# XiaoJiang-Phy/TensorCrossInterpolation.jl

Hardware: AMD Instinct MI355X
Metric: rrLU GFLOP/s at (m,n,r)=(8192,8192,256) (higher is better)
Workload: dtype f64

## Files before the change

include/tci_hip.h:

```cpp
#ifndef TCI_HIP_H
#define TCI_HIP_H

#include <stdint.h>

#ifdef __cplusplus
extern "C" {
#endif

#define TCI_OK 0
#define TCI_ERR_ARG 1
#define TCI_ERR_NAN 2
#define TCI_ERR_NONSQ 3
#define TCI_ERR_DEVICE 4
#define TCI_ERR_NOMEM 5
#define TCI_ERR_HOST 6

#define TCI_F_SUM 0
#define TCI_F_LORENTZ 1
#define TCI_F_TABLE 2
#define TCI_F_GAUSS 3
#define TCI_F_GAUSSMIX 4
#define TCI_F_QOSC 5
#define TCI_F_QEXP 6
#define TCI_F_TT 7
// ... 10 lines not shown
typedef int (*tci_exchange_fn)(void* user, int op, const void* d_send, void* d_recv, int64_t count);

int tci_ctx_create(int device, tci_ctx** out);
int tci_ctx_destroy(tci_ctx* ctx);
const char* tci_last_error(const tci_ctx* ctx);
void* tci_ctx_stream(tci_ctx* ctx);
int tci_ctx_synchronize(tci_ctx* ctx);
int tci_last_kernel_stats(tci_ctx* ctx, int family, double* total_ms, int64_t* launches);
int tci_last_kernel_units(tci_ctx* ctx, int family, double* total_ms, int64_t* launches, int64_t* units);
int tci_set_timing(tci_ctx* ctx, int enabled);
int tci_set_rrlu_flush(tci_ctx* ctx, int nb);
int tci_set_rrlu_epochs(tci_ctx* ctx, int epochs);
int tci_rrlu_epochs_for(tci_ctx* ctx, int64_t m, int64_t n);
int tci_set_rrlu_small(tci_ctx* ctx, int enabled);
int tci_set_rrlu_mid(tci_ctx* ctx, int enabled);
int tci_set_rrlu_persist(tci_ctx* ctx, int enabled);
int tci_rrlu_persist_faulted(tci_ctx* ctx);
int tci_set_shard_exchange(tci_ctx* ctx, int mode);
int tci_last_shard_exchange(tci_ctx* ctx);
int tci_set_rrlu_shadow(tci_ctx* ctx, int enabled);
int tci_rrlu_shadow_bytes(void);
int tci_set_c128_shadow(tci_ctx* ctx, int enabled);

int tci_set_dense_mfma(tci_ctx* ctx, int mask);

int tci_func_create(tci_ctx* ctx, int kind, const double* params, int64_t nparams,
                    const int32_t* localdims, int32_t L, tci_func** out);
int tci_func_destroy(tci_func* f);

typedef int (*tci_host_fn)(void* user, const int32_t* I, int64_t m, int32_t nl, const int32_t* J,
// ... 181 lines not shown
```

tensorcrossinterpolation.jl_amd/csrc/tci_abi.cpp:

```cpp
#include <hip/hip_runtime.h>
#include <stdint.h>
#include <stdlib.h>
#include <string.h>

#include <algorithm>
#include <cstddef>
#include <cmath>
#include <string>
#include <thread>
#include <vector>

#include <rccl/rccl.h>

#include "../../include/tci_hip.h"
#include "tci_internal.h"

using tci::Cand;
using tci::FuncDev;
using tci::RrluState;

struct tci_ctx {
    int device = 0;
    hipStream_t stream = nullptr;
    std::string err;
// ... 10 lines not shown
    double* xbuf = nullptr;
    size_t capX = 0;
    double* ybuf = nullptr;
    size_t capY = 0;
    int flush_every = 10;
    int epochs = 0;
    int serpentine = 1;
    int shadow = 1;
    int pass_gridx = 1;
    int pass_griddiv = 1;
    float* sbuf = nullptr;
    size_t capS = 0;
    int small_path = 1;
    int mid_path = 1;
    int mid_faulted = 0;
    int persist = 0;
    int persist_faulted = 0;
    int persist_kinds = 3;
    int persist_maxpass = 1 << 30;
    unsigned* esync = nullptr;
    size_t capEsync = 0;
    int dense = tci::kDenseAll;
    int c128_nb = -1;
    int c128_sh = 1;
    int ncu = 0;
    double* colbuf = nullptr;
    size_t capColbuf = 0;
    unsigned* bar = nullptr;
    int* fault = nullptr;
    int* flag = nullptr;
// ... 516 lines not shown
    g.lds = 0;
    if (shadow) {
        g.lds = round_up(m, 16);
        if ((st = ensure(c, &c->sbuf, &c->capS, (size_t)(g.lds * n)))) return st;
        g.S = c->sbuf;
        if ((st = zero_shadow_pad(c, g.lds, m, n))) return st;
    }
    const int grid = tci::argmax_grid(mi, ni, -1, g.cb,
                                      std::min(std::max(std::max(c->ncu, 1) * c->pass_gridx / c->pass_griddiv, 8), kMaxGrid));
    const int epochs = (shadow && tci::shadow_two_level() && nb >= 2 && nb <= 15 &&
                        tci::refresh_fits(g.lds, n))
                           ? std::max(1, std::min(rrlu_epochs(c, m, n), tci::kMaxPendR / nb)) : 1;
    const int nbx = nb * epochs;
    g.nbs = nb;
    g.pe = g.ps = 0;
    g.Asrc = dsrc;
    g.ldsrc = ldsrc;
    tci::launch_pass(c->stream, 0, false, shadow, g, grid);
    g.Asrc = nullptr;
    struct Sched {
        int PE, PS;
        bool last, flush, refresh;
    };
    auto sched = [&](int64_t kk, int64_t te, int64_t ts) {
        Sched s;
        s.PE = (int)(kk - te) + 1;
        s.PS = (int)(kk - ts) + 1;
        s.last = kk + 1 >= mr;
        s.flush = s.PE >= nbx && !s.last;
        s.refresh = !s.flush && epochs > 1 && s.PS >= nb && !s.last;
        return s;
    };
// ... 4 lines not shown
    int64_t nlaunch = 0;
    if (persist) {
        const size_t slots = (size_t)mr / 2 + 2;
        if ((st = ensure(c, &c->esync, &c->capEsync, slots * tci::kEpochSlot))) return st;
        HIPCHK(c, hipMemsetAsync(c->esync, 0, slots * tci::kEpochSlot * sizeof(unsigned), c->stream));
    }
    int64_t k = 0, chunk = 2, te = 0, ts = 0;
    StopPoll poll(c, c->st);
    for (;;) {
        while (k < mr) {
            const int64_t kend = std::min<int64_t>(k + chunk, mr);
            int64_t kk = k;
            while (kk < kend) {
                const Sched s = sched(kk, te, ts);
                const bool ro = !s.flush && !s.refresh && !s.last;
                if (persist && ro && kk >= 1 && s.PS <= tci::kEpochMaxP && (c->persist_kinds & (s.PE > s.PS ? 2 : 1))) {
                    int np = 1;
                    for (; np < c->persist_maxpass; ++np) {
                        const Sched t = sched(kk + np, te, ts);
                        if (t.flush || t.refresh || t.last || t.PS > tci::kEpochMaxP) break;
                    }
                    if (np >= 2) {
                        g.k = (int)kk;
                        g.pe = s.PE;
                        g.ps = s.PS;
                        g.selk = (int)(kk + 1);
                        const bool sampled = nlaunch % 3 == 0;
                        ev_begin(c, s.PE > s.PS ? tci_ctx::kFamEpoch + 1 : tci_ctx::kFamEpoch, sampled, -1, np);
                        tci::launch_pass_epoch(c->stream, g, grid, np, c->serpentine,
                                               c->esync + (size_t)nlaunch * tci::kEpochSlot, ptimeout);
// ... 33 lines not shown
        persist = false;
        k = c->hst->np - 1;
        te = ts = 0;
        for (int64_t q = 0; q < k; ++q) {
            const Sched s = sched(q, te, ts);
            if (s.flush) te = ts = q + 1;
            if (s.refresh) ts = q + 1;
        }
        HIPCHK(c, hipMemsetAsync(&c->st->done, 0, sizeof(int32_t), c->stream));
        chunk = 2;
        poll = StopPoll(c, c->st);
    }
    int64_t np = c->hst->np;
    double err = c->hst->error;
    if (np >= std::min(m, n)) err = 0.0;
    *np_out = np;
    *err_out = err;
    return TCI_OK;
}

int extract_LU(tci_ctx* c, int64_t m, int64_t n, int64_t np, int leftorth, bool wantL, bool wantU) {
    if (np <= 0) return TCI_OK;
    int st;
    if (wantL && (st = ensure(c, &c->dL, &c->capL, (size_t)(m * np)))) return st;
    if (wantU && (st = ensure(c, &c->dU, &c->capU, (size_t)(np * n)))) return st;
    HIPCHK(c, hipMemsetAsync(c->flag, 0, sizeof(int), c->stream));
    tci::launch_extract(c->stream, c->Lp, m, c->Up, c->ldUp, c->pivv, c->rowperm, c->colperm, (int)m,
                        (int)n, (int)np, leftorth, wantL ? c->dL : nullptr, m, wantU ? c->dU : nullptr,
                        np, c->flag);
    HIPCHK(c, hipMemcpyAsync(c->hflag, c->flag, sizeof(int), hipMemcpyDeviceToHost, c->stream));
// ... 322 lines not shown
    if (hipGetDeviceCount(&ndev) != hipSuccess || ndev <= 0) return TCI_ERR_DEVICE;
    if (device < 0 || device >= ndev) return TCI_ERR_ARG;
    tci_ctx* c = new tci_ctx();
    c->device = device;
    if (const char* e = getenv("TCI_RRLU_NB")) c->flush_every = std::max(1, std::min(atoi(e), tci::kMaxPend));
    if (const char* e = getenv("TCI_RRLU_SERP")) c->serpentine = atoi(e) != 0;
    if (const char* e = getenv("TCI_RRLU_EPOCHS")) c->epochs = std::max(0, std::min(atoi(e), tci::kMaxPendR));
    if (const char* e = getenv("TCI_RRLU_SHADOW")) c->shadow = atoi(e) != 0;
    if (const char* e = getenv("TCI_PASS_GRIDX")) c->pass_gridx = std::max(1, std::min(atoi(e), 8));
    if (const char* e = getenv("TCI_PASS_GRIDDIV")) c->pass_griddiv = std::max(1, std::min(atoi(e), 16));
    if (const char* e = getenv("TCI_RRLU_SMALL")) c->small_path = atoi(e) != 0;
    if (const char* e = getenv("TCI_SWEEP_SMALL")) c->small_sweep = atoi(e) != 0;
    if (const char* e = getenv("TCI_SW_LUWAVE")) c->sw_lu_wave = atoi(e) != 0;
    if (const char* e = getenv("TCI_SW_LAZYU")) c->sw_lazy_union = atoi(e) != 0;
    if (const char* e = getenv("TCI_RRLU_MID")) c->mid_path = atoi(e) != 0;
    if (const char* e = getenv("TCI_RRLU_PERSIST")) c->persist = tci::kEpochGrid && atoi(e) != 0;
    if (const char* e = getenv("TCI_SHARD_EXCHANGE")) c->sh_exchange = std::max(0, std::min(atoi(e), 2));
    if (const char* e = getenv("TCI_EPOCH_KINDS")) c->persist_kinds = atoi(e);
    if (const char* e = getenv("TCI_EPOCH_MAXPASS")) c->persist_maxpass = std::max(1, atoi(e));
    if (const char* e = getenv("TCI_C128_NB")) c->c128_nb = std::max(0, std::min(atoi(e), tci::kMaxPend - 1));
    if (const char* e = getenv("TCI_C128_SH")) c->c128_sh = atoi(e) != 0;
    if (const char* e = getenv("TCI_DENSE_MFMA")) c->dense = std::max(0, std::min(atoi(e), (int)tci::kDenseAll));
    {
        hipDeviceProp_t prop;
        if (hipGetDeviceProperties(&prop, device) == hipSuccess) c->ncu = prop.multiProcessorCount;
    }
    if (hipSetDevice(device) != hipSuccess ||
        hipStreamCreateWithFlags(&c->stream, hipStreamNonBlocking) != hipSuccess) {
        delete c;
        return TCI_ERR_DEVICE;
// ... 100 lines not shown

int tci_set_c128_shadow(tci_ctx* c, int enabled) {
    c->c128_sh = enabled != 0;
    return TCI_OK;
}

int tci_set_dense_mfma(tci_ctx* c, int mask) {
    if (!c || mask < 0 || mask > tci::kDenseAll) return TCI_ERR_ARG;
    c->dense = mask;
    return TCI_OK;
}

int tci_set_rrlu_mid(tci_ctx* c, int enabled) {
    c->mid_path = enabled != 0;
    c->mid_faulted = 0;
    return TCI_OK;
}

int tci_set_rrlu_persist(tci_ctx* c, int enabled) {
    if (!c) return TCI_ERR_ARG;
    if (enabled < 0 || enabled > 2) return set_err(c, TCI_ERR_ARG, "persist must be 0, 1 or 2 (test mode)");
    if (enabled && !tci::kEpochGrid)
        return set_err(c, TCI_ERR_ARG, "the persistent epoch grid is not built (default; -DTCI_EPOCH_GRID=1)");
    c->persist = enabled;
    c->persist_faulted = 0;
    return TCI_OK;
}

int tci_rrlu_persist_faulted(tci_ctx* c) { return c ? c->persist_faulted : -1; }

// ... 1796 lines not shown
```

tensorcrossinterpolation.jl_amd/csrc/tci_rrlu.hip:

```cpp
#include <hip/hip_runtime.h>
#include <math.h>
#include <stdint.h>

#include <type_traits>

#include "tci_internal.h"
#include "tci_smalllu.h"

#ifndef TCI_PASS2_U
#define TCI_PASS2_U 4
#endif
#ifndef TCI_SH_HALF
#define TCI_SH_HALF 1
#endif
#ifndef TCI_PASS_SH_U
#define TCI_PASS_SH_U 2
#endif
#ifndef TCI_SH_MFMA
#define TCI_SH_MFMA TCI_SH_HALF
#endif
#ifndef TCI_SH_NT
#define TCI_SH_NT 0
#endif
#ifndef TCI_SH_TIGHT
// ... 506 lines not shown
template <bool COH, typename T>
__device__ __forceinline__ T ldc(const T* p) {
    if constexpr (COH)
        return __hip_atomic_load((gptr<T>)(p), __ATOMIC_RELAXED, __HIP_MEMORY_SCOPE_AGENT);
    else
        return *p;
}
template <bool COH, typename T>
__device__ __forceinline__ void stc(T* p, T v) {
    if constexpr (COH)
        __hip_atomic_store((gptr<T>)(p), v, __ATOMIC_RELAXED, __HIP_MEMORY_SCOPE_AGENT);
    else
        *p = v;
}

template <int P, bool FLUSH, bool SH, bool COH = false>
__device__ __forceinline__ bool pass2_body(const PassK& g, const SelArgs& sel,
                                           P2Lds<(P > 0 ? P : 1)>& L, CandR& best,
                                           unsigned long long (&pt)[8]) {
    RrluState* st = sel.st;
    const int32_t* rowpos = sel.rowpos;
    const int32_t* colpos = sel.colpos;
    double* __restrict__ A = g.A;
    const int64_t lda = g.lda;
    const int m = g.m, n = g.n, k = g.k, cb = g.cb, rev = g.rev, leftorth = g.leftorth;
    double* __restrict__ X = g.X;
    double* __restrict__ Y = g.Y;
    const int64_t ldx = g.ldx, ldy = g.ldy;
    constexpr int U = TCI_PASS2_U;
    static_assert(U <= 8 && 8 % U == 0, "U must divide every column-tile width");
    constexpr int PP = P > 0 ? P : 1;
// ... 1 lines not shown
    int* cpos_s = L.cpos;
    int* cnt = L.cnt;
    const int lane = threadIdx.x & 63, wave = threadIdx.x >> 6;
    const int slice = wave % kP2Slices, rep = wave / kP2Slices;
    const int tiles_r = (m + kRowsPerTile - 1) / kRowsPerTile;
    const int tiles_c = (n + cb - 1) / cb;
    const int nq = gridDim.x / tiles_r;
    const int wid = xcd_spread(blockIdx.x, gridDim.x);
    const int tr = wid % tiles_r;
    const int q = rev ? nq - 1 - wid / tiles_r : wid / tiles_r;
    const int ntc = q < tiles_c ? (tiles_c - 1 - q) / nq + 1 : 0;
    const int G = kP2StageCols / cb;
    const int r0 = tr * kRowsPerTile + slice * 128 + 2 * lane;
    const bool rowok = r0 < m, pair = r0 + 1 < m;
    double* const base = A + (rowok ? r0 : 0);
    const bool cpy = P == 0 && g.Asrc != nullptr;
    const double* const sbase = cpy ? g.Asrc + (rowok ? r0 : 0) : base;
    const int64_t slda = cpy ? g.ldsrc : lda;
    auto chunk_col = [&](int g0, int h) -> int {
        const int it = g0 + (h * U) / cb;
        return (q + (rev ? ntc - 1 - it : it) * nq) * cb + (h * U) % cb;
    };
    auto load_chunk = [&](int g0, int h, double2 (&v)[U]) {
        const int j = chunk_col(g0, h);
#pragma unroll
        for (int u = 0; u < U; ++u) {
            const double2* pa = reinterpret_cast<const double2*>(sbase + (int64_t)min(j + u, n - 1) * slda);
            if constexpr (FLUSH && TCI_FLUSH_NTL) {
                typedef double dv2 __attribute__((ext_vector_type(2)));
                const dv2 w = __builtin_nontemporal_load(reinterpret_cast<const dv2*>(pa));
                v[u] = double2{w.x, w.y};
// ... 27 lines not shown
    if (rep < nch0) load_chunk(0, rep, va);
    if (rep + kP2Reps < nch0) load_chunk(0, rep + kP2Reps, vb);
    if (st->done) return false;
    int a = 0, b = 0;
    double piv = 1.0;
    if (P > 0) {
        a = (int)st->p;
        b = (int)st->q;
        piv = st->pval;
    }
    const bool in0 = rp0 > k, in1 = rp1 > k;
    const bool active = in0 || in1;
    [[maybe_unused]] const double shs =
        (SH && kShHalf && P > 0) ? sh_scale(sh_bound(sel.pivvals, FLUSH ? k + 1 : 0)) : 1.0;
    if constexpr (P > 0) {
        const double2 cb2 = *reinterpret_cast<const double2*>(A + (rowok ? r0 : 0) + (int64_t)b * lda);
        double xk0 = cb2.x, xk1 = cb2.y;
#pragma unroll
        for (int s = 0; s < P - 1; ++s) {
            const double yv = Y[(int64_t)s * ldy + b];
            xk0 = __dsub_rn(xk0, __dmul_rn(x0[s], yv));
            xk1 = __dsub_rn(xk1, __dmul_rn(x1[s], yv));
        }
        if (leftorth) {
            xk0 = xk0 / piv;
            xk1 = xk1 / piv;
        }
        x0[P - 1] = xk0;
        x1[P - 1] = xk1;
        if (q == 0 && rep == 0) {
            double* xs = X + (int64_t)(P - 1) * ldx;
            if (in0) {
                stc<COH>(xs + r0, xk0);
                g.Lp[r0 + (int64_t)k * g.ldl] = xk0;
            }
            if (in1) {
                stc<COH>(xs + r0 + 1, xk1);
                g.Lp[r0 + 1 + (int64_t)k * g.ldl] = xk1;
            }
        }
    }
    PPROF(1);
    const bool wact = (SH && kShHalf && P > 0) || __any(active);
    for (int g0 = 0; g0 < ntc; g0 += G) {
        const int gn = min(G, ntc - g0);
        const int nch = gn * cb / U;
        if (g0 > 0) {
            jst = stage_col(g0);
            cpst = (jst >= 0 && jst < n) ? colpos[jst] : -1;
            if (wact) {
                if (rep < nch) load_chunk(g0, rep, va);
                if (rep + kP2Reps < nch) load_chunk(g0, rep + kP2Reps, vb);
            }
            __syncthreads();
        }
        if (jst >= 0) {
            const int lc = threadIdx.x;
            cpos_s[lc] = cpst;
            if (P > 0 && cpst > k) {
                double yk = A[a + (int64_t)jst * lda];
#pragma unroll
                for (int s = 0; s < P - 1; ++s) {
                    const double ysv = Y[(int64_t)s * ldy + jst];
                    ys[lc * PP + s] = ysv;
                    yk = __dsub_rn(yk, __dmul_rn(X[(int64_t)s * ldx + a], ysv));
                }
                if (!leftorth) yk = yk / piv;
                ys[lc * PP + P - 1] = yk;
                if (tr == 0) {
                    stc<COH>(Y + (int64_t)(P - 1) * ldy + jst, yk);
                    g.Up[k + (int64_t)jst * g.ldu] = yk;
                }
            }
        }
        if (threadIdx.x < kP2Slices) cnt[threadIdx.x] = 2 * kP2Reps;
        __syncthreads();
        if (g0 == 0) PPROF(2);
        if (!wact) continue;
        auto column = [&](double2 v, int lc, int j) {
            const int cp = cpos_s[lc];
            if (cp <= k) return;
            if (P == 0 && cpy && rowok) {
                double* pw = base + (int64_t)j * lda;
                if (pair)
                    *reinterpret_cast<double2*>(pw) = v;
                else
                    pw[0] = v.x;
            }
            if constexpr (SH && kShHalf && !FLUSH && P > 0) {
                if (rowok && kShU8) {
                    uint8_t* ps = reinterpret_cast<uint8_t*>(g.S) + r0 + (int64_t)j * g.lds;
                    const uint32_t c0 = sh_u8((float)(v.x * shs));
                    if (pair)
                        *reinterpret_cast<uint16_t*>(ps) = (uint16_t)(c0 | sh_u8((float)(v.y * shs)) << 8);
                    else
                        ps[0] = (uint8_t)c0;
// ... 80 lines not shown
        };
        int h0 = rep, h1 = rep + kP2Reps;
        while (h0 < nch) {
            process(h0, va);
            h0 = grab();
            if (h0 < nch) load_chunk(g0, h0, va);
            if (h1 >= nch) break;
            process(h1, vb);
            h1 = grab();
            if (h1 < nch) load_chunk(g0, h1, vb);
        }
    }
    return true;
}

template <int P, bool FLUSH, bool SH>
__global__ __launch_bounds__(kP2Threads) void k_pass2(PassK g, SelArgs sel) {
    __shared__ P2Lds<(P > 0 ? P : 1)> L;
    [[maybe_unused]] unsigned long long pt[8] = {0, 0, 0, 0, 0, 0, 0, 0};
    PPROF(0);
    CandR best = cand_none();
    if (!pass2_body<P, FLUSH, SH>(g, sel, L, best, pt)) return;
    PPROF(3);
    pass_tail<kP2Threads>(best, sel, g.cand, pt, g.m, P, (int)FLUSH);
}

template <int P>
__device__ __forceinline__ bool pass_sh_body(const PassK& g, const SelArgs& sel, P2Lds<P>& L,
                                             CandR& best, float eps, double shs,
                                             unsigned long long (&pt)[8]) {
    RrluState* st = sel.st;
    const int32_t* colpos = sel.colpos;
    const int m = g.m, n = g.n, k = g.k, cb = g.cb, rev = g.rev;
    const int64_t lda = g.lda, ldx = g.ldx, ldy = g.ldy, lds = g.lds;
    constexpr int U = TCI_PASS_SH_U;
    const int lane = threadIdx.x & 63, wave = threadIdx.x >> 6;
    const int slice = wave % kShSlices, rep = wave / kShSlices;
// ... 978 lines not shown

constexpr int kXHalf = 256;
#ifndef TCI_XSTAGE
#define TCI_XSTAGE 128
#endif
#ifndef TCI_PX_EXP
#define TCI_PX_EXP 0
#endif
constexpr int kXStage = TCI_XSTAGE;
#ifndef TCI_PX_DRAIN
#define TCI_PX_DRAIN 1
#endif
#ifndef TCI_XU
#define TCI_XU 4
#endif
constexpr int kXU = TCI_XU;
static_assert(kXU == 4 || kXU == 8, "chunks of 4 or 8 columns (cb is a multiple of 8)");
constexpr int kXSlices = kXHalf / 128;
constexpr int kXReps = kP2Threads / 64 / kXSlices;
template <int NT>
struct PxGeom {
    static constexpr int Half = NT == 1024 ? 256 : 128;
    static constexpr int Tile = 2 * Half;
    static constexpr int Slices = Half / 128;
    static constexpr int Reps = NT / 64 / Slices;
};
template <int NT>
struct alignas(16) PxLdsT {
    alignas(16) double xs[kMaxPendR * PxGeom<NT>::Half];
    alignas(16) double ys[kMaxPendR * kXStage];
    double xa[kMaxPendR];
    double yb[kMaxPendR];
    int cpos[kXStage];
    int cnt[PxGeom<NT>::Slices];
};
using PxLds = PxLdsT<kP2Threads>;

template <int MODE, bool COH = false, int NT = kP2Threads>
__device__ __forceinline__ bool passx_body(const PassK& g, const SelArgs& sel, PxLdsT<NT>& L, CandR& best,
                                           unsigned long long (&pt)[8]) {
    constexpr int kXHalf = PxGeom<NT>::Half, kXSlices = PxGeom<NT>::Slices, kXReps = PxGeom<NT>::Reps;
    constexpr int kRowsPerTile = PxGeom<NT>::Tile, kP2Threads = NT;
    RrluState* st = sel.st;
    const int32_t* rowpos = sel.rowpos;
    const int32_t* colpos = sel.colpos;
    double* __restrict__ A = g.A;
    const int64_t lda = g.lda, ldx = g.ldx, ldy = g.ldy;
    const int m = g.m, n = g.n, k = g.k, cb = g.cb, rev = g.rev, leftorth = g.leftorth;
    const int P = g.pe;
    const int lane = threadIdx.x & 63, wave = __builtin_amdgcn_readfirstlane(threadIdx.x >> 6);
    const int slice = wave % kXSlices, rep = wave / kXSlices;
    const int tiles_r = (m + kRowsPerTile - 1) / kRowsPerTile;
    const int tiles_c = (n + cb - 1) / cb;
    const int nq = gridDim.x / tiles_r;
    const int wid = xcd_spread(blockIdx.x, gridDim.x);
    const int tr = wid % tiles_r;
    const int q = rev ? nq - 1 - wid / tiles_r : wid / tiles_r;
    const int ntc = q < tiles_c ? (tiles_c - 1 - q) / nq + 1 : 0;
    const int G = kXStage / cb;
    const int cbs = __builtin_ctz(cb);
    auto col_of = [&](int g0, int lc) -> int {
        const int it = g0 + (lc >> cbs);
// ... 20 lines not shown
                const int e = threadIdx.x + u * kP2Threads, s = e / kXHalf, rr = e - s * kXHalf;
                v[u] = g.X[(int64_t)s * ldx + min(hb + rr, m - 1)];
                if (!(s < P - 1 && hb + rr < m)) v[u] = 0.0;
            }
#pragma unroll
            for (int u = 0; u < kPer; ++u) {
                const int e = threadIdx.x + u * kP2Threads;
                if (e < (P - 1) * kXHalf) L.xs[e] = v[u];
            }
        }
        __syncthreads();
        if (threadIdx.x < kXHalf) {
            const int rr = threadIdx.x, r = hb + rr;
            double xk = 0.0;
            if (r < m) {
                xk = A[r + (int64_t)b * lda];
                for (int s = 0; s < P - 1; ++s) xk = __dsub_rn(xk, __dmul_rn(L.xs[s * kXHalf + rr], L.yb[s]));
                if (leftorth) xk = xk / piv;
                if (q == 0 && rowpos[r] > k) {
                    stc<COH>(g.X + (int64_t)(P - 1) * ldx + r, xk);
                    g.Lp[r + (int64_t)k * g.ldl] = xk;
                }
            }
            L.xs[(P - 1) * kXHalf + rr] = xk;
        }
        const int lr = slice * 128 + 2 * lane;
        const int r0 = hb + lr;
        const bool rowok = r0 < m, pair = r0 + 1 < m;
        const int rp0 = rowok ? rowpos[r0] : -1, rp1 = pair ? rowpos[r0 + 1] : -1;
        const bool in0 = rp0 > k, in1 = rp1 > k;
        const bool wact = MODE != 0 || __any(in0 || in1);
// ... 9 lines not shown
                double v[kPer];
#pragma unroll
                for (int u = 0; u < kPer; ++u) {
                    const int s = s0 + u * (kP2Threads / kXStage);
                    v[u] = g.Y[(int64_t)s * ldy + j];
                    if (!(s < P - 1 && lc < gcols)) v[u] = 0.0;
                }
#pragma unroll
                for (int u = 0; u < kPer; ++u) {
                    const int s = s0 + u * (kP2Threads / kXStage);
                    if (s < P - 1) L.ys[s * kXStage + lc] = v[u];
                }
            }
            const int lcs = threadIdx.x, js = lcs < gcols ? col_of(g0, lcs) : 0;
            const int cps = (lcs < gcols && js < n) ? colpos[js] : -1;
            const double ypr = (lcs < gcols && cps > k) ? A[a + (int64_t)js * lda] : 0.0;
            __syncthreads();
            if (lcs < gcols) {
                L.cpos[lcs] = cps;
                if (cps > k) {
                    double yk = ypr;
                    for (int s = 0; s < P - 1; ++s) yk = __dsub_rn(yk, __dmul_rn(L.xa[s], L.ys[s * kXStage + lcs]));
                    if (!leftorth) yk = yk / piv;
                    L.ys[(P - 1) * kXStage + lcs] = yk;
                    if (tr == 0 && half == 0) {
                        stc<COH>(g.Y + (int64_t)(P - 1) * ldy + js, yk);
                        g.Up[k + (int64_t)js * g.ldu] = yk;
                    }
                }
            }
            if (threadIdx.x < kXSlices) L.cnt[threadIdx.x] = 2 * kXReps;
            __syncthreads();
            if (g0 == 0 && half == 0) PPROF(2);
            if (!wact) continue;
            auto load_chunk = [&](int h, double2 (&v)[kXU]) {
                const int j0 = col_of(g0, h * kXU);
#pragma unroll
                for (int u = 0; u < kXU; ++u) {
                    const double* colp = A + (int64_t)min(j0 + u, n - 1) * lda;
                    const double2* pa = reinterpret_cast<const double2*>(colp + roff);
                    if constexpr (MODE == 1 && TCI_FLUSH_NTL) {
                        typedef double dv2 __attribute__((ext_vector_type(2)));
                        const dv2 w = __builtin_nontemporal_load(reinterpret_cast<const dv2*>(pa));
                        v[u] = double2{w.x, w.y};
                    } else {
                        v[u] = *pa;
                    }
                }
            };
            auto process = [&](int h, double2 (&v)[kXU]) {
                int cp[kXU];
                bool any = false;
#pragma unroll
                for (int u = 0; u < kXU; ++u) {
                    cp[u] = __builtin_amdgcn_readfirstlane(L.cpos[h * kXU + u]);
                    any |= cp[u] > k;
                }
                if (!any) return;
                const int j0 = col_of(g0, h * kXU);
#pragma unroll 2
                for (int s = 0; s < P; ++s) {
#if TCI_PX_EXP & 1
                    const dv2 x = dv2{1.0 + s, 0.5 * s};
#else
                    const dv2 x = *reinterpret_cast<const dv2*>(
                        __builtin_assume_aligned(&L.xs[s * kXHalf + lr], 16));
#endif
                    double y[kXU];
#pragma unroll
                    for (int u = 0; u < kXU; u += 2) {
#if TCI_PX_EXP & 2
// ... 5 lines not shown
                        y[u] = yy.x;
                        y[u + 1] = yy.y;
                    }
#pragma unroll
                    for (int u = 0; u < kXU; ++u) {
                        v[u].x = __dsub_rn(v[u].x, __dmul_rn(x.x, y[u]));
                        v[u].y = __dsub_rn(v[u].y, __dmul_rn(x.y, y[u]));
                    }
                }
                double mx0 = 0.0, mx1 = 0.0;
#pragma unroll
                for (int u = 0; u < kXU; ++u) {
                    if (cp[u] <= k) continue;
                    const int j = j0 + u;
                    if constexpr (MODE == 1) {
                        if (in0 || in1) {
                            double2* pa = reinterpret_cast<double2*>(A + (int64_t)j * lda + roff);
                            if (!in1) {
                                pa->x = v[u].x;
                            } else if (!in0) {
                                pa->y = v[u].y;
                            } else {
                                typedef double dv2 __attribute__((ext_vector_type(2)));
                                dv2 w = {v[u].x, v[u].y};
                                __builtin_nontemporal_store(w, reinterpret_cast<dv2*>(pa));
                            }
                        }
                    }
                    if constexpr (MODE != 0 && kShU8) {
                        if (rowok) {
                            uint8_t* ps = reinterpret_cast<uint8_t*>(g.S) + (int64_t)j * g.lds + roff;
                            const uint32_t c0 = in0 ? sh_u8((float)(v[u].x * shs)) : kShU8Zero;
                            if (pair)
                                *reinterpret_cast<uint16_t*>(ps) =
                                    (uint16_t)(c0 | (in1 ? sh_u8((float)(v[u].y * shs)) : kShU8Zero) << 8);
                            else
// ... 54 lines not shown
            while (h0 < nch) {
                process(h0, va);
                h0 = grab();
                if (h0 < nch) load_chunk(h0, va);
                if (h1 >= nch) break;
                process(h1, vb);
                h1 = grab();
                if (h1 < nch) load_chunk(h1, vb);
            }
#endif
        }
    }
    return true;
}

template <int MODE, int NT = kP2Threads>
__global__ __launch_bounds__(NT) __attribute__((amdgpu_waves_per_eu(4))) void k_pass_x(PassK g, SelArgs sel) {
    __shared__ PxLdsT<NT> L;
    [[maybe_unused]] unsigned long long pt[8] = {0, 0, 0, 0, 0, 0, 0, 0};
    PPROF(0);
    CandR best = cand_none();
    if (!passx_body<MODE, false, NT>(g, sel, L, best, pt)) return;
    PPROF(3);
    pass_tail<NT>(best, sel, g.cand, pt, g.m, g.pe, MODE);
}

template <int P, bool EXT, bool RF, bool RT = false>
__global__ __launch_bounds__(kP2Threads) void k_pass_mf(PassK g, SelArgs sel) {
    __shared__ union {
        P2Lds<P> x;
        P2MfLds<P, EXT> f;
        typename std::conditional<(EXT || RF), PxLds, char>::type px;
    } L;
    [[maybe_unused]] unsigned long long pt[8] = {0, 0, 0, 0, 0, 0, 0, 0};
    PPROF(0);
#if TCI_PASS_PROF
    if (threadIdx.x == 0) g_exam_lds = 0;
// ... 209 lines not shown
}

int shadow_elem_bytes() { return kShU8 ? 1 : kShHalf ? 2 : 4; }
bool shadow_two_level() { return kShHalf && TCI_SH_MFMA; }

int argmax_grid(int m, int n, int k, int cb, int max_grid) {
    (void)k;
    const long long tiles_r = m > 0 ? (m + kRowsPerTile - 1) / kRowsPerTile : 1;
    const long long tiles_c = n > 0 ? (n + cb - 1) / cb : 1;
    long long nq = max_grid / tiles_r;
    if (nq > tiles_c) nq = tiles_c;
    if (nq < 1) nq = 1;
    return (int)(tiles_r * nq);
}

template <int P>
static void launch_pass_p(hipStream_t s, bool flush, bool shadow, const PassArgs& g, int grid, int kind) {
    const SelArgs sel{g.rowpos, g.colpos, g.rowphys, g.colphys, g.pivvals, g.st,
                      g.ticket, g.reltol, g.abstol,  g.selk,    g.lout, g.pc_off};
    const PassK a{g.A,  g.lda, g.m,  g.n,   g.k,        g.X,    g.ldx, g.Y,   g.ldy,
                  g.Lp, g.ldl, g.Up, g.ldu, g.leftorth, g.cand, g.cb,  g.rev, g.S, g.lds,
                  g.pe, g.ps, g.nbs, g.Asrc, g.ldsrc};
    if (shadow && kShHalf) {
        if (P == 0)
            hipLaunchKernelGGL((k_pass2<0, false, false>), dim3(grid), dim3(kP2Threads), 0, s, a, sel);
        else if (flush)
            hipLaunchKernelGGL((k_pass2<P, true, true>), dim3(grid), dim3(kP2Threads), 0, s, a, sel);
        else if (P == 1 && g.k == 0)
            hipLaunchKernelGGL((k_pass2<1, false, true>), dim3(grid), dim3(kP2Threads), 0, s, a, sel);
        else if constexpr (P > 0) {
            const bool ext = g.pe > g.ps, rf = kind == 2;
            if constexpr (TCI_SH_MFMA && P <= kMfMaxP) {
                if (ext && rf)
                    hipLaunchKernelGGL((k_pass_mf<P, true, true>), dim3(grid), dim3(kP2Threads), 0, s, a, sel);
                else if (ext && TCI_PASS_ONEP)
                    hipLaunchKernelGGL((k_pass_mf<kEpochMaxP, true, false, true>), dim3(grid), dim3(kP2Threads), 0, s, a, sel);
                else if (ext)
                    hipLaunchKernelGGL((k_pass_mf<P, true, false>), dim3(grid), dim3(kP2Threads), 0, s, a, sel);
                else if (rf)
                    hipLaunchKernelGGL((k_pass_mf<P, false, true>), dim3(grid), dim3(kP2Threads), 0, s, a, sel);
                else
                    hipLaunchKernelGGL((k_pass_mf<P, false, false>), dim3(grid), dim3(kP2Threads), 0, s, a, sel);
            } else if constexpr (kShU8) {
// ... 4 lines not shown
        }
    } else if (shadow && !kShHalf) {
        if constexpr (!kShHalf) {
            if (flush || P == 0)
                hipLaunchKernelGGL((k_pass2<P, (P > 0), true>), dim3(grid), dim3(kP2Threads), 0, s, a, sel);
            else if constexpr (P > 0)
                hipLaunchKernelGGL((k_pass_sh<P>), dim3(grid), dim3(kP2Threads), 0, s, a, sel);
        }
    } else if (flush) {
        hipLaunchKernelGGL((k_pass2<P, true, false>), dim3(grid), dim3(kP2Threads), 0, s, a, sel);
    } else {
        hipLaunchKernelGGL((k_pass2<P, false, false>), dim3(grid), dim3(kP2Threads), 0, s, a, sel);
    }
}

#ifndef TCI_PASSX_MIN
#define TCI_PASSX_MIN 12
#endif

void launch_pass(hipStream_t s, int P, bool flush, bool shadow, const PassArgs& g, int grid, int kind) {
    if (kind < 0) kind = flush ? 1 : 0;
    PassArgs h = g;
    if (h.pe <= 0) h.pe = h.ps = P;
    if (kind == 1 && shadow && kShHalf && h.pe >= TCI_PASSX_MIN) {
        const SelArgs sel{h.rowpos, h.colpos, h.rowphys, h.colphys, h.pivvals, h.st,
                          h.ticket, h.reltol, h.abstol,  h.selk,    h.lout, h.pc_off};
        const PassK a{h.A,  h.lda, h.m,  h.n,   h.k,        h.X,    h.ldx, h.Y,   h.ldy,
                      h.Lp, h.ldl, h.Up, h.ldu, h.leftorth, h.cand, h.cb,  h.rev, h.S, h.lds,
                      h.pe, h.ps, h.nbs, h.Asrc, h.ldsrc};
        static const int px_nt = [] {
            const char* e = getenv("TCI_PASSX_NT");
            return e ? atoi(e) : 512;
        }();
        const int tiles_r = (h.m + kRowsPerTile - 1) / kRowsPerTile;
        const int nq = grid / tiles_r;
        const int tiles_r2 = (h.m + PxGeom<512>::Tile - 1) / PxGeom<512>::Tile;
        if (px_nt == 512 && (int64_t)tiles_r2 * nq <= kMaxPassGrid)
            hipLaunchKernelGGL((k_pass_x<1, 512>), dim3(tiles_r2 * nq), dim3(512), 0, s, a, sel);
        else
            hipLaunchKernelGGL((k_pass_x<1>), dim3(grid), dim3(kP2Threads), 0, s, a, sel);
        return;
    }
    const int PP = kind == 1 || !(shadow && kShHalf) ? h.pe : h.ps;
    switch (PP) {
#define TCI_PASS_CASE(p) \
    case p: launch_pass_p<p>(s, kind == 1, shadow, h, grid, kind); break;
        TCI_PASS_CASE(0) TCI_PASS_CASE(1) TCI_PASS_CASE(2) TCI_PASS_CASE(3) TCI_PASS_CASE(4)
        TCI_PASS_CASE(5) TCI_PASS_CASE(6) TCI_PASS_CASE(7) TCI_PASS_CASE(8) TCI_PASS_CASE(9)
        TCI_PASS_CASE(10) TCI_PASS_CASE(11) TCI_PASS_CASE(12) TCI_PASS_CASE(13) TCI_PASS_CASE(14)
        TCI_PASS_CASE(15) TCI_PASS_CASE(16)
#undef TCI_PASS_CASE
    default: break;
// ... 662 lines not shown
```

tensorcrossinterpolation.jl_amd/tci_amd/_lib.py:

```python
import atexit
import ctypes as C
import os
import threading
import weakref

import numpy as np

_HERE = os.path.dirname(os.path.abspath(__file__))
LIB_PATH = os.environ.get("TCI_HIP_LIB", os.path.join(os.path.dirname(_HERE), "lib", "libtci_hip.so"))

TCI_OK, TCI_ERR_ARG, TCI_ERR_NAN, TCI_ERR_NONSQ, TCI_ERR_DEVICE, TCI_ERR_NOMEM, TCI_ERR_HOST = range(7)

i64p = np.ctypeslib.ndpointer(dtype=np.int64, flags="C_CONTIGUOUS")
i32p = np.ctypeslib.ndpointer(dtype=np.int32, flags="C_CONTIGUOUS")
f64p = np.ctypeslib.ndpointer(dtype=np.float64, flags="C_CONTIGUOUS")
vp = C.c_void_p
dbl = C.c_double
i64 = C.c_int64
i32 = C.c_int32
pi64 = C.POINTER(C.c_int64)
pdbl = C.POINTER(C.c_double)


class TCIError(RuntimeError):
# ... 17 lines not shown
    "tci_last_error": ([vp], C.c_char_p),
    "tci_ctx_stream": ([vp], vp),
    "tci_ctx_synchronize": ([vp], C.c_int),
    "tci_last_kernel_stats": ([vp, C.c_int, pdbl, pi64], C.c_int),
    "tci_last_kernel_units": ([vp, C.c_int, pdbl, pi64, pi64], C.c_int),
    "tci_set_rrlu_persist": ([vp, C.c_int], C.c_int),
    "tci_rrlu_persist_faulted": ([vp], C.c_int),
    "tci_set_shard_exchange": ([vp, C.c_int], C.c_int),
    "tci_last_shard_exchange": ([vp], C.c_int),
    "tci_set_timing": ([vp, C.c_int], C.c_int),
    "tci_set_rrlu_flush": ([vp, C.c_int], C.c_int),
    "tci_set_rrlu_epochs": ([vp, C.c_int], C.c_int),
    "tci_rrlu_epochs_for": ([vp, i64, i64], C.c_int),
    "tci_set_rrlu_small": ([vp, C.c_int], C.c_int),
    "tci_set_rrlu_mid": ([vp, C.c_int], C.c_int),
    "tci_set_rrlu_shadow": ([vp, C.c_int], C.c_int),
    "tci_rrlu_shadow_bytes": ([], C.c_int),
    "tci_set_c128_shadow": ([vp, C.c_int], C.c_int),
    "tci_set_dense_mfma": ([vp, C.c_int], C.c_int),
    "tci_func_create": ([vp, C.c_int, vp, i64, i32p, i32, C.POINTER(vp)], C.c_int),
    "tci_func_destroy": ([vp], C.c_int),
    "tci_func_create_host": ([vp, vp, vp, i32p, i32, C.POINTER(vp)], C.c_int),
    "tci_func_create_c128": ([vp, vp, i32, vp, i32, C.POINTER(vp)], C.c_int),
    "tci_batcheval_h": ([vp, vp, vp, i64, i32, vp, i64, i32, i32, vp, i64, pdbl], C.c_int),
    "tci_batcheval_d": ([vp, vp, vp, i64, i32, vp, i64, i32, i32, vp, i64, pdbl], C.c_int),
    "tci_batcheval_dd": ([vp, vp, vp, i64, i32, vp, i64, i32, i32, vp, i64, vp], C.c_int),
    "tci_batcheval_da": ([vp, vp, vp, i64, i32, vp, i64, i32, i32, vp, i64, vp], C.c_int),
    "tci_rrlu_h": ([vp, vp, i64, i64, i64, i64, dbl, dbl, C.c_int, vp, vp, vp, vp, i64, pi64, pdbl],
                   C.c_int),
    "tci_rrlu_c128_h": ([vp, vp, i64, i64, i64, i64, dbl, dbl, C.c_int, vp, vp, vp, vp, i64, pi64, pdbl,
# ... 241 lines not shown
```

Baseline: 2650.

## Read rrLU input directly from source until first flush, skipping initial copy

Before the first write-back, the rrLU passes now read matrix entries straight from the caller's source buffer rather than first copying the whole input into the working array. The first flush pass reads the source and writes every column back, including pivoted and untouched entries, so the working copy becomes complete at that point. A fallback copy runs if factorization stops before the first flush. This removes one full read and write of the 8192x8192 f64 matrix. In exchange it adds new template kernel variants and extra raw-copy stores inside the flush pass.

```diff
diff --git a/include/tci_hip.h b/include/tci_hip.h
--- a/include/tci_hip.h
+++ b/include/tci_hip.h
@@ -48,6 +48,7 @@
 int tci_rrlu_epochs_for(tci_ctx* ctx, int64_t m, int64_t n);
 int tci_set_rrlu_small(tci_ctx* ctx, int enabled);
 int tci_set_rrlu_mid(tci_ctx* ctx, int enabled);
+int tci_set_rrlu_src_direct(tci_ctx* ctx, int enabled);
 int tci_set_rrlu_persist(tci_ctx* ctx, int enabled);
 int tci_rrlu_persist_faulted(tci_ctx* ctx);
 int tci_set_shard_exchange(tci_ctx* ctx, int mode);
diff --git a/tensorcrossinterpolation.jl_amd/csrc/tci_abi.cpp b/tensorcrossinterpolation.jl_amd/csrc/tci_abi.cpp
--- a/tensorcrossinterpolation.jl_amd/csrc/tci_abi.cpp
+++ b/tensorcrossinterpolation.jl_amd/csrc/tci_abi.cpp
@@ -48,6 +48,7 @@
     int small_path = 1;
     int mid_path = 1;
     int mid_faulted = 0;
+    int src_direct = 1;
     int persist = 0;
     int persist_faulted = 0;
     int persist_kinds = 3;
@@ -594,8 +595,15 @@
     const int nbx = nb * epochs;
     g.nbs = nb;
     g.pe = g.ps = 0;
-    g.Asrc = dsrc;
+    const bool srcdirect = dsrc && c->src_direct && mr > nbx && shadow && tci::shadow_elem_bytes() <= 2 &&
+                           ldsrc % 4 == 0;
+    auto on_input = [&](bool in) {
+        g.A = in ? const_cast<double*>(dsrc) : dA;
+        g.lda = in ? ldsrc : lda;
+    };
+    g.Asrc = srcdirect ? nullptr : dsrc;
     g.ldsrc = ldsrc;
+    on_input(srcdirect);
     tci::launch_pass(c->stream, 0, false, shadow, g, grid);
     g.Asrc = nullptr;
     struct Sched {
@@ -630,6 +638,8 @@
             while (kk < kend) {
                 const Sched s = sched(kk, te, ts);
                 const bool ro = !s.flush && !s.refresh && !s.last;
+                on_input(srcdirect && te == 0 && !s.flush);
+                g.Asrc = srcdirect && te == 0 && s.flush ? dsrc : nullptr;
                 if (persist && ro && kk >= 1 && s.PS <= tci::kEpochMaxP && (c->persist_kinds & (s.PE > s.PS ? 2 : 1))) {
                     int np = 1;
                     for (; np < c->persist_maxpass; ++np) {
@@ -693,6 +703,8 @@
     int64_t np = c->hst->np;
     double err = c->hst->error;
     if (np >= std::min(m, n)) err = 0.0;
+    if (srcdirect && np < nbx)
+        if ((st = copy_input())) return st;
     *np_out = np;
     *err_out = err;
     return TCI_OK;
@@ -1045,6 +1057,7 @@
     if (const char* e = getenv("TCI_SW_LUWAVE")) c->sw_lu_wave = atoi(e) != 0;
     if (const char* e = getenv("TCI_SW_LAZYU")) c->sw_lazy_union = atoi(e) != 0;
     if (const char* e = getenv("TCI_RRLU_MID")) c->mid_path = atoi(e) != 0;
+    if (const char* e = getenv("TCI_RRLU_SRCDIRECT")) c->src_direct = atoi(e) != 0;
     if (const char* e = getenv("TCI_RRLU_PERSIST")) c->persist = tci::kEpochGrid && atoi(e) != 0;
     if (const char* e = getenv("TCI_SHARD_EXCHANGE")) c->sh_exchange = std::max(0, std::min(atoi(e), 2));
     if (const char* e = getenv("TCI_EPOCH_KINDS")) c->persist_kinds = atoi(e);
@@ -1175,6 +1188,12 @@
 int tci_set_rrlu_mid(tci_ctx* c, int enabled) {
     c->mid_path = enabled != 0;
     c->mid_faulted = 0;
+    return TCI_OK;
+}
+
+int tci_set_rrlu_src_direct(tci_ctx* c, int enabled) {
+    if (!c) return TCI_ERR_ARG;
+    c->src_direct = enabled != 0;
     return TCI_OK;
 }
 
diff --git a/tensorcrossinterpolation.jl_amd/csrc/tci_rrlu.hip b/tensorcrossinterpolation.jl_amd/csrc/tci_rrlu.hip
--- a/tensorcrossinterpolation.jl_amd/csrc/tci_rrlu.hip
+++ b/tensorcrossinterpolation.jl_amd/csrc/tci_rrlu.hip
@@ -544,7 +544,7 @@
         *p = v;
 }
 
-template <int P, bool FLUSH, bool SH, bool COH = false>
+template <int P, bool FLUSH, bool SH, bool COH = false, bool SRC = false>
 __device__ __forceinline__ bool pass2_body(const PassK& g, const SelArgs& sel,
                                            P2Lds<(P > 0 ? P : 1)>& L, CandR& best,
                                            unsigned long long (&pt)[8]) {
@@ -576,7 +576,9 @@
     const int r0 = tr * kRowsPerTile + slice * 128 + 2 * lane;
     const bool rowok = r0 < m, pair = r0 + 1 < m;
     double* const base = A + (rowok ? r0 : 0);
-    const bool cpy = P == 0 && g.Asrc != nullptr;
+    static_assert(!SRC || (FLUSH && P > 0), "only a write-back reads the input in place of A");
+    const bool cpy = SRC || (P == 0 && g.Asrc != nullptr);
+    const double* const Ain = cpy ? g.Asrc : A;
     const double* const sbase = cpy ? g.Asrc + (rowok ? r0 : 0) : base;
     const int64_t slda = cpy ? g.ldsrc : lda;
     auto chunk_col = [&](int g0, int h) -> int {
@@ -634,7 +636,7 @@
     [[maybe_unused]] const double shs =
         (SH && kShHalf && P > 0) ? sh_scale(sh_bound(sel.pivvals, FLUSH ? k + 1 : 0)) : 1.0;
     if constexpr (P > 0) {
-        const double2 cb2 = *reinterpret_cast<const double2*>(A + (rowok ? r0 : 0) + (int64_t)b * lda);
+        const double2 cb2 = *reinterpret_cast<const double2*>(sbase + (int64_t)b * slda);
         double xk0 = cb2.x, xk1 = cb2.y;
 #pragma unroll
         for (int s = 0; s < P - 1; ++s) {
@@ -661,7 +663,7 @@
         }
     }
     PPROF(1);
-    const bool wact = (SH && kShHalf && P > 0) || __any(active);
+    const bool wact = (SH && kShHalf && P > 0) || SRC || __any(active);
     for (int g0 = 0; g0 < ntc; g0 += G) {
         const int gn = min(G, ntc - g0);
         const int nch = gn * cb / U;
@@ -678,7 +680,7 @@
             const int lc = threadIdx.x;
             cpos_s[lc] = cpst;
             if (P > 0 && cpst > k) {
-                double yk = A[a + (int64_t)jst * lda];
+                double yk = Ain[a + (int64_t)jst * slda];
 #pragma unroll
                 for (int s = 0; s < P - 1; ++s) {
                     const double ysv = Y[(int64_t)s * ldy + jst];
@@ -699,7 +701,20 @@
         if (!wact) continue;
         auto column = [&](double2 v, int lc, int j) {
             const int cp = cpos_s[lc];
-            if (cp <= k) return;
+            auto copy_raw = [&](bool w0, bool w1) {
+                double* pw = base + (int64_t)j * lda;
+                if (w0 && w1)
+                    *reinterpret_cast<double2*>(pw) = v;
+                else if (w0)
+                    pw[0] = v.x;
+                else if (w1)
+                    pw[1] = v.y;
+            };
+            if (cp <= k) {
+                if (SRC && cp >= 0) copy_raw(rowok, pair);
+                return;
+            }
+            if (SRC && !(in0 && in1)) copy_raw(rowok && !in0, pair && !in1);
             if (P == 0 && cpy && rowok) {
                 double* pw = base + (int64_t)j * lda;
                 if (pair)
@@ -810,13 +825,13 @@
     return true;
 }
 
-template <int P, bool FLUSH, bool SH>
+template <int P, bool FLUSH, bool SH, bool SRC = false>
 __global__ __launch_bounds__(kP2Threads) void k_pass2(PassK g, SelArgs sel) {
     __shared__ P2Lds<(P > 0 ? P : 1)> L;
     [[maybe_unused]] unsigned long long pt[8] = {0, 0, 0, 0, 0, 0, 0, 0};
     PPROF(0);
     CandR best = cand_none();
-    if (!pass2_body<P, FLUSH, SH>(g, sel, L, best, pt)) return;
+    if (!pass2_body<P, FLUSH, SH, false, SRC>(g, sel, L, best, pt)) return;
     PPROF(3);
     pass_tail<kP2Threads>(best, sel, g.cand, pt, g.m, P, (int)FLUSH);
 }
@@ -1825,6 +1840,9 @@
 #ifndef TCI_XU
 #define TCI_XU 4
 #endif
+#ifndef TCI_SRC_NT
+#define TCI_SRC_NT 2
+#endif
 constexpr int kXU = TCI_XU;
 static_assert(kXU == 4 || kXU == 8, "chunks of 4 or 8 columns (cb is a multiple of 8)");
 constexpr int kXSlices = kXHalf / 128;
@@ -1847,9 +1865,10 @@
 };
 using PxLds = PxLdsT<kP2Threads>;
 
-template <int MODE, bool COH = false, int NT = kP2Threads>
+template <int MODE, bool COH = false, int NT = kP2Threads, bool SRC = false>
 __device__ __forceinline__ bool passx_body(const PassK& g, const SelArgs& sel, PxLdsT<NT>& L, CandR& best,
                                            unsigned long long (&pt)[8]) {
+    static_assert(!SRC || MODE == 1, "only the write-back reads the input");
     constexpr int kXHalf = PxGeom<NT>::Half, kXSlices = PxGeom<NT>::Slices, kXReps = PxGeom<NT>::Reps;
     constexpr int kRowsPerTile = PxGeom<NT>::Tile, kP2Threads = NT;
     RrluState* st = sel.st;
@@ -1857,6 +1876,8 @@
     const int32_t* colpos = sel.colpos;
     double* __restrict__ A = g.A;
     const int64_t lda = g.lda, ldx = g.ldx, ldy = g.ldy;
+    const double* const Ain = SRC ? g.Asrc : A;
+    const int64_t ldin = SRC ? g.ldsrc : lda;
     const int m = g.m, n = g.n, k = g.k, cb = g.cb, rev = g.rev, leftorth = g.leftorth;
     const int P = g.pe;
     const int lane = threadIdx.x & 63, wave = __builtin_amdgcn_readfirstlane(threadIdx.x >> 6);
@@ -1907,7 +1928,7 @@
             const int rr = threadIdx.x, r = hb + rr;
             double xk = 0.0;
             if (r < m) {
-                xk = A[r + (int64_t)b * lda];
+                xk = Ain[r + (int64_t)b * ldin];
                 for (int s = 0; s < P - 1; ++s) xk = __dsub_rn(xk, __dmul_rn(L.xs[s * kXHalf + rr], L.yb[s]));
                 if (leftorth) xk = xk / piv;
                 if (q == 0 && rowpos[r] > k) {
@@ -1947,7 +1968,7 @@
             }
             const int lcs = threadIdx.x, js = lcs < gcols ? col_of(g0, lcs) : 0;
             const int cps = (lcs < gcols && js < n) ? colpos[js] : -1;
-            const double ypr = (lcs < gcols && cps > k) ? A[a + (int64_t)js * lda] : 0.0;
+            const double ypr = (lcs < gcols && cps > k) ? Ain[a + (int64_t)js * ldin] : 0.0;
             __syncthreads();
             if (lcs < gcols) {
                 L.cpos[lcs] = cps;
@@ -1970,9 +1991,9 @@
                 const int j0 = col_of(g0, h * kXU);
 #pragma unroll
                 for (int u = 0; u < kXU; ++u) {
-                    const double* colp = A + (int64_t)min(j0 + u, n - 1) * lda;
+                    const double* colp = Ain + (int64_t)min(j0 + u, n - 1) * ldin;
                     const double2* pa = reinterpret_cast<const double2*>(colp + roff);
-                    if constexpr (MODE == 1 && TCI_FLUSH_NTL) {
+                    if constexpr (MODE == 1 && TCI_FLUSH_NTL && (!SRC || (TCI_SRC_NT & 1))) {
                         typedef double dv2 __attribute__((ext_vector_type(2)));
                         const dv2 w = __builtin_nontemporal_load(reinterpret_cast<const dv2*>(pa));
                         v[u] = double2{w.x, w.y};
@@ -1988,6 +2009,18 @@
                 for (int u = 0; u < kXU; ++u) {
                     cp[u] = __builtin_amdgcn_readfirstlane(L.cpos[h * kXU + u]);
                     any |= cp[u] > k;
+                }
+                [[maybe_unused]] auto copy_raw = [&](int j, bool w0, bool w1) {
+                    const double* pi = Ain + (int64_t)j * ldin + roff;
+                    double* pw = A + (int64_t)j * lda + roff;
+                    if (w0) pw[0] = pi[0];
+                    if (w1) pw[1] = pi[1];
+                };
+                if constexpr (SRC) {
+                    const int jc = col_of(g0, h * kXU);
+#pragma unroll
+                    for (int u = 0; u < kXU; ++u)
+                        if (cp[u] <= k && cp[u] >= 0) copy_raw(jc + u, rowok, pair);
                 }
                 if (!any) return;
                 const int j0 = col_of(g0, h * kXU);
@@ -2023,12 +2056,17 @@
                     if (cp[u] <= k) continue;
                     const int j = j0 + u;
                     if constexpr (MODE == 1) {
+                        if constexpr (SRC) {
+                            if (!(in0 && in1)) copy_raw(j, rowok && !in0, pair && !in1);
+                        }
                         if (in0 || in1) {
                             double2* pa = reinterpret_cast<double2*>(A + (int64_t)j * lda + roff);
                             if (!in1) {
                                 pa->x = v[u].x;
                             } else if (!in0) {
                                 pa->y = v[u].y;
+                            } else if constexpr (SRC && !(TCI_SRC_NT & 2)) {
+                                *pa = v[u];
                             } else {
                                 typedef double dv2 __attribute__((ext_vector_type(2)));
                                 dv2 w = {v[u].x, v[u].y};
@@ -2113,13 +2151,13 @@
     return true;
 }
 
-template <int MODE, int NT = kP2Threads>
+template <int MODE, int NT = kP2Threads, bool SRC = false>
 __global__ __launch_bounds__(NT) __attribute__((amdgpu_waves_per_eu(4))) void k_pass_x(PassK g, SelArgs sel) {
     __shared__ PxLdsT<NT> L;
     [[maybe_unused]] unsigned long long pt[8] = {0, 0, 0, 0, 0, 0, 0, 0};
     PPROF(0);
     CandR best = cand_none();
-    if (!passx_body<MODE, false, NT>(g, sel, L, best, pt)) return;
+    if (!passx_body<MODE, false, NT, SRC>(g, sel, L, best, pt)) return;
     PPROF(3);
     pass_tail<NT>(best, sel, g.cand, pt, g.m, g.pe, MODE);
 }
@@ -2359,6 +2397,10 @@
     return (int)(tiles_r * nq);
 }
 
+#ifndef TCI_PASSX_MIN
+#define TCI_PASSX_MIN 12
+#endif
+
 template <int P>
 static void launch_pass_p(hipStream_t s, bool flush, bool shadow, const PassArgs& g, int grid, int kind) {
     const SelArgs sel{g.rowpos, g.colpos, g.rowphys, g.colphys, g.pivvals, g.st,
@@ -2369,9 +2411,15 @@
     if (shadow && kShHalf) {
         if (P == 0)
             hipLaunchKernelGGL((k_pass2<0, false, false>), dim3(grid), dim3(kP2Threads), 0, s, a, sel);
-        else if (flush)
+        else if (flush) {
+            if constexpr (P > 0 && P < TCI_PASSX_MIN) {
+                if (g.Asrc) {
+                    hipLaunchKernelGGL((k_pass2<P, true, true, true>), dim3(grid), dim3(kP2Threads), 0, s, a, sel);
+                    return;
+                }
+            }
             hipLaunchKernelGGL((k_pass2<P, true, true>), dim3(grid), dim3(kP2Threads), 0, s, a, sel);
-        else if (P == 1 && g.k == 0)
+        } else if (P == 1 && g.k == 0)
             hipLaunchKernelGGL((k_pass2<1, false, true>), dim3(grid), dim3(kP2Threads), 0, s, a, sel);
         else if constexpr (P > 0) {
             const bool ext = g.pe > g.ps, rf = kind == 2;
@@ -2406,10 +2454,6 @@
     }
 }
 
-#ifndef TCI_PASSX_MIN
-#define TCI_PASSX_MIN 12
-#endif
-
 void launch_pass(hipStream_t s, int P, bool flush, bool shadow, const PassArgs& g, int grid, int kind) {
     if (kind < 0) kind = flush ? 1 : 0;
     PassArgs h = g;
@@ -2427,7 +2471,13 @@
         const int tiles_r = (h.m + kRowsPerTile - 1) / kRowsPerTile;
         const int nq = grid / tiles_r;
         const int tiles_r2 = (h.m + PxGeom<512>::Tile - 1) / PxGeom<512>::Tile;
-        if (px_nt == 512 && (int64_t)tiles_r2 * nq <= kMaxPassGrid)
+        const bool nt512 = px_nt == 512 && (int64_t)tiles_r2 * nq <= kMaxPassGrid;
+        if (h.Asrc) {
+            if (nt512)
+                hipLaunchKernelGGL((k_pass_x<1, 512, true>), dim3(tiles_r2 * nq), dim3(512), 0, s, a, sel);
+            else
+                hipLaunchKernelGGL((k_pass_x<1, kP2Threads, true>), dim3(grid), dim3(kP2Threads), 0, s, a, sel);
+        } else if (nt512)
             hipLaunchKernelGGL((k_pass_x<1, 512>), dim3(tiles_r2 * nq), dim3(512), 0, s, a, sel);
         else
             hipLaunchKernelGGL((k_pass_x<1>), dim3(grid), dim3(kP2Threads), 0, s, a, sel);
diff --git a/tensorcrossinterpolation.jl_amd/tci_amd/_lib.py b/tensorcrossinterpolation.jl_amd/tci_amd/_lib.py
--- a/tensorcrossinterpolation.jl_amd/tci_amd/_lib.py
+++ b/tensorcrossinterpolation.jl_amd/tci_amd/_lib.py
@@ -55,6 +55,7 @@
     "tci_rrlu_epochs_for": ([vp, i64, i64], C.c_int),
     "tci_set_rrlu_small": ([vp, C.c_int], C.c_int),
     "tci_set_rrlu_mid": ([vp, C.c_int], C.c_int),
+    "tci_set_rrlu_src_direct": ([vp, C.c_int], C.c_int),
     "tci_set_rrlu_shadow": ([vp, C.c_int], C.c_int),
     "tci_rrlu_shadow_bytes": ([], C.c_int),
     "tci_set_c128_shadow": ([vp, C.c_int], C.c_int),
```

After: 2649. Within noise of the previous version (-0.0%).
